# alinjar1996/manipulator_mujoco

Measured on NVIDIA B200. Metric: rollout env-steps/sec (CEM iteration, UR5e+Hand-E scene, 4096 samples x 100 steps per GPU), higher is better.
Workload: dtype f32

## Files before the change

### manipulator_mujoco_b200/csrc/rollout_core.h

```cpp
#pragma once
#include "kmodel.h"
#include "warp_dsl.h"

#ifndef CEMK_SYNC_EVERY
#define CEMK_SYNC_EVERY 1
#endif
#define KM_NC_FAST (KW == 16 ? 20 : 24)
#define KM_NPASS (KM_MAXRPAIR / KW)
#define KM_NC_TOT 48
#define KM_OVF_STRIDE 80
#define KM_NC_BIG 48
#ifndef CEMK_ROW_UNROLL
#define CEMK_ROW_UNROLL 1
#endif
constexpr int kRowUnroll = CEMK_ROW_UNROLL;
#define MJ_MINVAL 1e-15f
#define MJ_MINIMP 0.0001f
#define MJ_MAXIMP 0.9999f

struct LaneRegs {
  float cost_c;
  int nact, off;
  int actmask;
  int farprev;
  int tri;
  float acc[9];
  float h[KM_NV];
#ifdef CEMK_EMU
  float hrow[KM_NV];
#endif
  float td;
  float f0, f1, f2;
};

template <int NC>
struct WarpSmemT {
  static constexpr int NROW = KM_NL + 4 * NC;
  float qpos[16], qvel[12], warm[12];
  float lpos[KM_NL][4], lquat[KM_NL][4], lmat[KM_NL][12];
  float cdof[KM_NL][8];
  float bmat[12];
  float Mr[KM_NL][KM_NL];
  union {
    struct { float capA[KM_MAXCAP][4], capB[KM_MAXCAP][4]; };
    float H[KM_NV][KM_NV];
  };
  float fs[12], as[12], qacc[12], Ma[12], grad[12], search[12];
  int ncon, nrow, nlim, flags;
  union {
    struct { float cinert[KM_NL][12], crb[KM_NL][12], cvel[KM_NL][8], cdofdot[KM_NL][8], cfrc[KM_NL][8]; };
    struct { float rD[NROW], rAref[NROW], rJaref[NROW], rJv[NROW]; };
    struct {
      unsigned short nlist[KM_MAXNEAR];
      float nprev[(KM_MAXSBOX + 1) * KW][2];
    };
  };
  float cgeo[NC][16];
  union {
    float cJ[NC][36];
    struct {
      float bstage[KM_MAXBPAIR][4][4], bnrm[KM_MAXBPAIR][4];
      union {
        struct { float bbR[12], bbc[4], bbsz[2][4], bbrf[4][4], bben[4][4], bbpoly[2][8][4], bbpref[8][4]; };
        struct { float estage[KW][16], eres[KW][8]; };
      };
    };
  };
  float cd[2][NC][3];
  int limdof[KM_NL];
  float limsign[KM_NL];
  float* ovf;
  float* ovf_pad;

  template <bool SP> KMEM float* geo(int c) const { return (!SP || c < NC) ? const_cast<float*>(cgeo[c]) : ovf + (c - NC) * KM_OVF_STRIDE; }
  template <bool SP> KMEM float* jac(int c) const { return (!SP || c < NC) ? const_cast<float*>(cJ[c]) : ovf + (c - NC) * KM_OVF_STRIDE + 16; }
  template <bool SP> KMEM float* dots(int set, int c) const {
    return (!SP || c < NC) ? const_cast<float*>(cd[set][c]) : ovf + (c - NC) * KM_OVF_STRIDE + 52 + 3 * set;
  }
  template <bool SP> KMEM float& row(const float* arr, int off, int r, int nl) const {
    const int rc = r - nl;
    return (!SP || rc < 4 * NC) ? const_cast<float*>(arr)[r] : ovf[((rc >> 2) - NC) * KM_OVF_STRIDE + off + (rc & 3)];
  }
  template <bool SP> KMEM float& D(int r, int nl) const { return row<SP>(rD, 58, r, nl); }
  template <bool SP> KMEM float& Aref(int r, int nl) const { return row<SP>(rAref, 62, r, nl); }
  template <bool SP> KMEM float& Jaref(int r, int nl) const { return row<SP>(rJaref, 66, r, nl); }
  template <bool SP> KMEM float& Jv(int r, int nl) const { return row<SP>(rJv, 70, r, nl); }
};

typedef WarpCtx<LaneRegs> Warp;

KFN int tri_entries(int lane) {
  int tri = 0;
  for (int q = 0; q < 32 / KW; ++q) {
    int e = lane + KW * q, i = 0, j = e;
    if (e < KM_NL * (KM_NL + 1) / 2) { while (j > i) { j -= i + 1; ++i; } } else { i = 15; j = 15; }
    tri |= (i | (j << 4)) << (8 * q);
  }
  return tri;
}
KFN void cold_warp(Warp& W, int bar, int nthr) {
#ifdef CEMK_EMU
  std::memset((void*)&W, 0, sizeof(Warp));
  W.race = g_emu_race;
  for (int l = 0; l < KW; ++l) W.regs[l].tri = tri_entries(l);
  (void)bar; (void)nthr;
#else
  W.lane = threadIdx.x & (KW - 1);
  W.shift = (threadIdx.x & 31) & ~(KW - 1);
  W.mask = KW_FULL << W.shift;
  W.bar = bar; W.nthr = nthr;
  W.regs.tri = tri_entries(W.lane);
#ifdef CEMK_PHASE_TIMING
  W.phase = 0; W.t0 = clock64(); W.stepflag = 0; W.nflag = 0;
  for (int i = 0; i < 24; ++i) { W.ph[i] = 0; W.phs[i] = 0; W.phc[i] = 0; }
  for (int i = 0; i < 24; ++i) W.ev[i] = 0;
#endif
#endif
}

KFN float dot3(const float* a, const float* b) { return a[0] * b[0] + a[1] * b[1] + a[2] * b[2]; }
KFN void cross3(float* r, const float* a, const float* b) {
  float x = a[1] * b[2] - a[2] * b[1], y = a[2] * b[0] - a[0] * b[2], z = a[0] * b[1] - a[1] * b[0];
  r[0] = x; r[1] = y; r[2] = z;
}
KFN void sub3(float* r, const float* a, const float* b) { r[0] = a[0] - b[0]; r[1] = a[1] - b[1]; r[2] = a[2] - b[2]; }
KFN void add3(float* r, const float* a, const float* b) { r[0] = a[0] + b[0]; r[1] = a[1] + b[1]; r[2] = a[2] + b[2]; }
KFN void madd3(float* r, const float* a, const float* b, float s) { r[0] = a[0] + s * b[0]; r[1] = a[1] + s * b[1]; r[2] = a[2] + s * b[2]; }
KFN void copy3(float* r, const float* a) { r[0] = a[0]; r[1] = a[1]; r[2] = a[2]; }
KFN float normalize3(float* a) {
  float n = sqrtf(dot3(a, a));
  if (n > 0.f) { float i = 1.f / n; a[0] *= i; a[1] *= i; a[2] *= i; } else { a[0] = a[1] = a[2] = 0.f; }
  return n;
}
KFN void mat_vec(float* r, const float* m, const float* v) {
  float x = m[0] * v[0] + m[1] * v[1] + m[2] * v[2], y = m[3] * v[0] + m[4] * v[1] + m[5] * v[2], z = m[6] * v[0] + m[7] * v[1] + m[8] * v[2];
  r[0] = x; r[1] = y; r[2] = z;
}
KFN void matT_vec(float* r, const float* m, const float* v) {
  float x = m[0] * v[0] + m[3] * v[1] + m[6] * v[2], y = m[1] * v[0] + m[4] * v[1] + m[7] * v[2], z = m[2] * v[0] + m[5] * v[1] + m[8] * v[2];
  r[0] = x; r[1] = y; r[2] = z;
}
KFN void quat_mul(float* r, const float* a, const float* b) {
  float w = a[0] * b[0] - a[1] * b[1] - a[2] * b[2] - a[3] * b[3];
  float x = a[0] * b[1] + a[1] * b[0] + a[2] * b[3] - a[3] * b[2];
  float y = a[0] * b[2] - a[1] * b[3] + a[2] * b[0] + a[3] * b[1];
  float z = a[0] * b[3] + a[1] * b[2] - a[2] * b[1] + a[3] * b[0];
  r[0] = w; r[1] = x; r[2] = y; r[3] = z;
// ... 173 lines not shown
      sub3(dv, sp.a, nb);
      const float d2 = dot3(dv, dv);
      if (d1 < d2) copy3(sp.a, na); else copy3(sp.b, nb);
    }
    float dir[3];
    sub3(dir, sp.a, sp.b);
    const bool deg = dot3(dir, dir) < 1e-6f;
    const float ed = normalize3(dir);
    const bool front = (eu * dir[u] < 0.f) && (ew * dir[w] < 0.f);
    const float epen = (!deg && front) ? r - ed : -1.f;
    if (epen > bpen) { bpen = epen; bdeg = deg; copy3(beax, dir); copy3(bec, sp.a); copy3(bcc, sp.b); }
  }
  const bool parallel = fabsf(dot3(beax, n)) > 0.99f && !bdeg;
  const bool has_edge = bpen > 0.f && (minface > 0.f ? bpen < minface : true) && !parallel;
  CapBoxEdge out;
  out.pen = has_edge ? bpen : 0.f;
#pragma unroll
  for (int q = 0; q < 3; ++q) { out.pos[q] = 0.5f * (bec[q] + bcc[q] + beax[q] * r); out.nrm[q] = beax[q]; }
  return out;
}
template <bool FULL, bool EDGES = true>
KFN int capsule_box_near(const float* a, const float* b, float r, const float* bsize, CapBoxOut& o, float* nface = nullptr) {
  float bests = fminf(a[0], b[0]) - bsize[0]; int bk = 0; float sg = 1.f;
  { float s = -fmaxf(a[0], b[0]) - bsize[0]; if (s > bests) { bests = s; sg = -1.f; } }
  { float s = fminf(a[1], b[1]) - bsize[1]; if (s > bests) { bests = s; bk = 1; sg = 1.f; } }
  { float s = -fmaxf(a[1], b[1]) - bsize[1]; if (s > bests) { bests = s; bk = 1; sg = -1.f; } }
  { float s = fminf(a[2], b[2]) - bsize[2]; if (s > bests) { bests = s; bk = 2; sg = 1.f; } }
  { float s = -fmaxf(a[2], b[2]) - bsize[2]; if (s > bests) { bests = s; bk = 2; sg = -1.f; } }
  float ak, au, aw, bk_, bu, bw, sk, su, sw;
  if (bk == 0)      { ak = a[0]; au = a[1]; aw = a[2]; bk_ = b[0]; bu = b[1]; bw = b[2]; sk = bsize[0]; su = bsize[1]; sw = bsize[2]; }
  else if (bk == 1) { ak = a[1]; au = a[2]; aw = a[0]; bk_ = b[1]; bu = b[2]; bw = b[0]; sk = bsize[1]; su = bsize[2]; sw = bsize[0]; }
  else              { ak = a[2]; au = a[0]; aw = a[1]; bk_ = b[2]; bu = b[0]; bw = b[1]; sk = bsize[2]; su = bsize[0]; sw = bsize[1]; }
  float t0 = 0.f, t1 = 1.f; bool both = false;
  {
    const float Lu = 2.f * sw, Lw = 2.f * su;
#define CEMK_CLIP(pa, pb, s, tau, L) { \
      float na_ = ((tau) * (pa) - (s)) * (L), nb_ = ((tau) * (pb) - (s)) * (L); \
      bool fa = na_ > 1e-6f, fb = nb_ > 1e-6f; \
      float den = (tau) * ((pb) - (pa)) * (L); \
      float tt = (-na_) / (den + (den == 0.f ? 1e-6f : 0.f)); \
      tt = fminf(fmaxf(tt, 0.f), 1.f); \
      if (fa) t0 = fmaxf(t0, tt); \
      if (fb) t1 = fminf(t1, tt); \
      both = both || (fa && fb); }
    CEMK_CLIP(au, bu, su, -1.f, Lu)
    CEMK_CLIP(aw, bw, sw, -1.f, Lw)
    CEMK_CLIP(au, bu, su, 1.f, Lu)
    CEMK_CLIP(aw, bw, sw, 1.f, Lw)
#undef CEMK_CLIP
  }
  bool mask = !both;
  if (!mask) { t0 = 0.f; t1 = 1.f; }
  {
    const float dk = bk_ - ak, du = bu - au, dw = bw - aw;
    if ((t1 - t0) * (dk * dk + du * du + dw * dw) < 0.f) mask = false;
  }
  const float h0 = sg * (ak + t0 * (bk_ - ak)) - r - sk, h1 = sg * (ak + t1 * (bk_ - ak)) - r - sk;
  o.dist[0] = mask ? h0 : 1.f;
  o.dist[1] = mask ? h1 : 1.f;
  const float nx = bk == 0 ? sg : 0.f, ny = bk == 1 ? sg : 0.f, nz = bk == 2 ? sg : 0.f;
  const int nout = ((fmaxf(a[0], b[0]) > bsize[0] || fminf(a[0], b[0]) < -bsize[0]) ? 1 : 0) +
                   ((fmaxf(a[1], b[1]) > bsize[1] || fminf(a[1], b[1]) < -bsize[1]) ? 1 : 0) +
                   ((fmaxf(a[2], b[2]) > bsize[2] || fminf(a[2], b[2]) < -bsize[2]) ? 1 : 0);
  if (FULL || nout >= 2) {
    const float l0[3] = {sg * (sk + 0.5f * h0), au + t0 * (bu - au), aw + t0 * (bw - aw)};
    const float l1[3] = {sg * (sk + 0.5f * h1), au + t1 * (bu - au), aw + t1 * (bw - aw)};
    if (bk == 0)      { o.pos[0][0] = l0[0]; o.pos[0][1] = l0[1]; o.pos[0][2] = l0[2]; o.pos[1][0] = l1[0]; o.pos[1][1] = l1[1]; o.pos[1][2] = l1[2]; }
    else if (bk == 1) { o.pos[0][1] = l0[0]; o.pos[0][2] = l0[1]; o.pos[0][0] = l0[2]; o.pos[1][1] = l1[0]; o.pos[1][2] = l1[1]; o.pos[1][0] = l1[2]; }
    else              { o.pos[0][2] = l0[0]; o.pos[0][0] = l0[1]; o.pos[0][1] = l0[2]; o.pos[1][2] = l1[0]; o.pos[1][0] = l1[1]; o.pos[1][1] = l1[2]; }
    o.nrm[0][0] = o.nrm[1][0] = -nx; o.nrm[0][1] = o.nrm[1][1] = -ny; o.nrm[0][2] = o.nrm[1][2] = -nz;
    if (EDGES && nout >= 2) {
      const CapBoxEdge e = capbox_edges(a[0], a[1], a[2], b[0], b[1], b[2], r, bsize[0], bsize[1], bsize[2], nx, ny, nz, fminf(-o.dist[0], -o.dist[1]));
      if (e.pen > 0.f) { o.dist[0] = -e.pen; copy3(o.pos[0], e.pos); copy3(o.nrm[0], e.nrm); }
    }
  }
  if (nface) { nface[0] = nx; nface[1] = ny; nface[2] = nz; }
  return nout;
}
struct EdgeEval { float epen, deg, dir[3], pa[3], pb[3]; };
KFN float pick3(const float* v, int k) { return k == 0 ? v[0] : (k == 1 ? v[1] : v[2]); }
KFN void unpick3(float* out, int k, int u, float vk, float vu, float vw) {
  out[0] = k == 0 ? vk : (u == 0 ? vu : vw); out[1] = k == 1 ? vk : (u == 1 ? vu : vw); out[2] = k == 2 ? vk : (u == 2 ? vu : vw);
}
KFN EdgeEval capbox_edge_lane(int e, const float* a, const float* b, float r, const float* bsize) {
  EdgeEval out;
  out.epen = -1.f; out.deg = 0.f;
  out.dir[0] = out.dir[1] = out.dir[2] = 0.f; out.pa[0] = out.pa[1] = out.pa[2] = 0.f; out.pb[0] = out.pb[1] = out.pb[2] = 0.f;
  const int k = e >> 2, u = k == 2 ? 0 : k + 1, w = k == 0 ? 2 : k - 1;
  const float eu = (e & 2) ? 1.f : -1.f, ew = (e & 1) ? 1.f : -1.f;
  const float ak = pick3(a, k), au = pick3(a, u), aw = pick3(a, w), bk = pick3(b, k), bu = pick3(b, u), bw = pick3(b, w);
  const float sk = pick3(bsize, k), su = pick3(bsize, u), sw = pick3(bsize, w);
  const float lou = fminf(au, bu), hiu = fmaxf(au, bu), low = fminf(aw, bw), hiw = fmaxf(aw, bw), lok = fminf(ak, bk), hik = fmaxf(ak, bk);
  const float cu = eu * su, cw = ew * sw;
  const float fu = eu > 0.f ? hiu - cu : cu - lou, fw = ew > 0.f ? hiw - cw : cw - low;
  const float gu = eu > 0.f ? lou - cu : cu - hiu, gw = ew > 0.f ? low - cw : cw - hiw;
  if (!(fu > 0.f && fw > 0.f && gu < r && gw < r && lok < sk + r && hik > -sk - r)) return out;
  const float abk = bk - ak, abu = bu - au, abw = bw - aw;
  const float den = abk * abk + abu * abu + abw * abw + 1e-6f;
  float dv[3] = {abk, abu, abw};
  const float hb = 0.5f * normalize3(dv);
  const float mk = ak + dv[0] * hb, mu = au + dv[1] * hb, mw = aw + dv[2] * hb;
  const float trk = -mk, tru = cu - mu, trw = cw - mw;
  const float dd = dv[0], dat = trk, dbt = dv[0] * trk + dv[1] * tru + dv[2] * trw;
  float ta = (-dat + dd * dbt) / (1.f - dd * dd + 1e-6f);
  float tb = dbt + ta * dd;
  ta = fminf(fmaxf(ta, -sk), sk);
  tb = fminf(fmaxf(tb, -hb), hb);
  float pa[3] = {ta, cu, cw}, pb[3] = {mk + dv[0] * tb, mu + dv[1] * tb, mw + dv[2] * tb};
  float t1 = ((pb[0] + sk) * (2.f * sk)) / (4.f * sk * sk + 1e-6f);
  t1 = fminf(fmaxf(t1, 0.f), 1.f);
  const float na[3] = {-sk + 2.f * sk * t1, cu, cw};
  float d[3];
  sub3(d, pb, na);
  const float d1 = dot3(d, d);
  float t2 = ((pa[0] - ak) * abk + (pa[1] - au) * abu + (pa[2] - aw) * abw) / den;
  t2 = fminf(fmaxf(t2, 0.f), 1.f);
  const float nb[3] = {ak + abk * t2, au + abu * t2, aw + abw * t2};
  sub3(d, pa, nb);
  const float d2 = dot3(d, d);
  if (d1 < d2) copy3(pa, na); else copy3(pb, nb);
  float dir[3];
  sub3(dir, pa, pb);
  const bool deg = dot3(dir, dir) < 1e-6f;
  const float ed = normalize3(dir);
  const bool front = (eu * dir[1] < 0.f) && (ew * dir[2] < 0.f);
  out.epen = (!deg && front) ? r - ed : -1.f;
  out.deg = deg ? 1.f : 0.f;
  unpick3(out.dir, k, u, dir[0], dir[1], dir[2]);
  unpick3(out.pa, k, u, pa[0], pa[1], pa[2]);
  unpick3(out.pb, k, u, pb[0], pb[1], pb[2]);
  return out;
}
template <bool FULL>
KFN void capsule_box(const float* A, const float* B, float r, const float* bpos, const float* bmat, const float* bsize, Contact2& c) {
  float a[3], b[3];
  capbox_local(A, B, bpos, bmat, a, b);
  c.dist[0] = 1.f; c.dist[1] = 1.f;
  if (capbox_far(a, b, r, bsize)) {
    if (FULL) { for (int j = 0; j < 2; ++j) { copy3(c.pos[j], bpos); c.nrm[j][0] = 1.f; c.nrm[j][1] = 0.f; c.nrm[j][2] = 0.f; } }
    return;
  }
  CapBoxOut o;
  capsule_box_near<FULL>(a, b, r, bsize, o);
  c.dist[0] = o.dist[0]; c.dist[1] = o.dist[1];
  if (FULL) {
#pragma unroll
    for (int j = 0; j < 2; ++j) {
      float w[3];
      mat_vec(w, bmat, o.pos[j]); add3(c.pos[j], w, bpos);
      mat_vec(c.nrm[j], bmat, o.nrm[j]);
      normalize3(c.nrm[j]);
    }
  }
}

KFN void manifold_points(int n, float poly[][3], const bool* mask, const float* nrm, int* idx) {
  float dm[16];
  for (int i = 0; i < n; ++i) dm[i] = mask[i] ? 0.f : -1e6f;
  int a = 0;
  for (int i = 1; i < n; ++i) if (dm[i] > dm[a]) a = i;
  int b = 0; float bv = 0.f;
  for (int i = 0; i < n; ++i) { float t[3]; sub3(t, poly[a], poly[i]); float v = dot3(t, t) + dm[i]; if (i == 0 || v > bv) { bv = v; b = i; } }
  float ab[3], t[3];
  sub3(t, poly[a], poly[b]); cross3(ab, nrm, t);
  int c = 0; float cv = 0.f;
  for (int i = 0; i < n; ++i) { float ap[3]; sub3(ap, poly[a], poly[i]); float v = fabsf(dot3(ap, ab)) + dm[i]; if (i == 0 || v > cv) { cv = v; c = i; } }
  float ac[3], bc[3];
  sub3(t, poly[a], poly[c]); cross3(ac, nrm, t);
  sub3(t, poly[b], poly[c]); cross3(bc, nrm, t);
  int dsel = 0; float dv = 0.f;
  for (int i = 0; i < n; ++i) {
    float bp[3], ap[3];
    sub3(bp, poly[b], poly[i]); sub3(ap, poly[a], poly[i]);
    float v = fmaxf(fabsf(dot3(bp, bc)), fabsf(dot3(ap, ac))) + dm[i] - ((i == a || i == b || i == c) ? 2e6f : 0.f);
    if (i == 0 || v > dv) { dv = v; dsel = i; }
  }
  idx[0] = a; idx[1] = b; idx[2] = c; idx[3] = dsel;
}
KFN void box_face(const float* s, int f, float v[4][3], float* n) {
  int k = f >> 1, u = (k + 1) % 3, w = (k + 2) % 3;
  float sg = (f & 1) ? -1.f : 1.f;
  n[0] = n[1] = n[2] = 0.f; n[k] = sg;
  const float su[4] = {-1.f, 1.f, 1.f, -1.f}, sw[4] = {-1.f, -1.f, 1.f, 1.f};
  for (int i = 0; i < 4; ++i) {
    int ii = (f & 1) ? 3 - i : i;
    v[i][k] = sg * s[k]; v[i][u] = su[ii] * s[u]; v[i][w] = sw[ii] * s[w];
  }
}
KNOINLINE int plane_box(const float* ppos, const float* pn, const float* bpos, const float* bmat, const float* bs, float out[4][4]) {
  float v[8][3], sup[8], t[3], pl[3], n[3], smax = -1e30f;
  bool mask[8]; int idx[4];
  sub3(t, ppos, bpos); matT_vec(pl, bmat, t); matT_vec(n, bmat, pn);
  for (int i = 0; i < 8; ++i) {
    v[i][0] = (i & 4 ? 1.f : -1.f) * bs[0]; v[i][1] = (i & 2 ? 1.f : -1.f) * bs[1]; v[i][2] = (i & 1 ? 1.f : -1.f) * bs[2];
    sub3(t, pl, v[i]); sup[i] = dot3(t, n); smax = fmaxf(smax, sup[i]);
  }
  float thr = fmaxf(0.f, smax - 1e-3f);
  for (int i = 0; i < 8; ++i) mask[i] = sup[i] > thr;
  manifold_points(8, v, mask, n, idx);
  int nact = 0;
  for (int k = 0; k < 4; ++k) {
    bool uniq = true;
    for (int q = 0; q < k; ++q) if (idx[q] == idx[k]) uniq = false;
    float w[3];
    mat_vec(w, bmat, v[idx[k]]); add3(w, w, bpos);
    float d = uniq ? -sup[idx[k]] : 1.f;
    madd3(out[k], w, pn, -0.5f * d);
    out[k][3] = d;
    nact += d < 0.f;
  }
  return nact;
}
template <int NC>
KNOINLINE void bb_edge_edge(WarpSmemT<NC>& S, bool act, int slot, int bl, float bn0, float bn1, float bn2, const float* s1, const float* s2,
                            const float* m2, const float* p2) {
// ... 981 lines not shown
      int rem = nearbits & ~R.farprev;
      if (rem) { pf0 = KFFS(rem) - 1; rem &= rem - 1; pf = 1; q00 = pd[(2 * pf0) * KW]; q01 = pd[(2 * pf0 + 1) * KW]; }
      if (rem) { pf1 = KFFS(rem) - 1; pf = 2; q10 = pd[(2 * pf1) * KW]; q11 = pd[(2 * pf1 + 1) * KW]; }
    }
    if (!io.first) {
#pragma unroll 1
      for (int rem = farbits & ~R.farprev; rem; rem &= rem - 1) {
        const int p = KFFS(rem) - 1;
        cc += fmaxf((1.f - 0.005f) * pd[(2 * p) * KW] - 1.f, 0.f) + fmaxf((1.f - 0.005f) * pd[(2 * p + 1) * KW] - 1.f, 0.f);
      }
    }
    if (io.collision_row) {
#pragma unroll 1
      for (int rem = farbits; rem; rem &= rem - 1) {
        const int sl = KP_SLOT(m.rp[(KFFS(rem) - 1) * KW + lane]);
        io.collision_row[sl] = 1.f; io.collision_row[sl + 1] = 1.f;
      }
    }
    R.off = nearbits | ((nearbits & R.farprev) << 16);
    R.farprev = farbits;
    float pv0 = 0.f, pv1 = 0.f;
    if (!io.first) { pv0 = pd[(2 * m.ncbpass) * KW]; pv1 = pd[(2 * m.ncbpass + 1) * KW]; }
#pragma unroll 1
    for (int p = m.ncbpass; p < KM_NPASS; ++p) {
      const int e = p * KW + lane;
      const int x = m.rp[e], ty = KP_TYPE(x);
      const float prev0 = pv0, prev1 = pv1;
      if (!io.first && p + 1 < KM_NPASS) { pv0 = pd[(2 * p + 2) * KW]; pv1 = pd[(2 * p + 3) * KW]; }
      if (ty == KP_NONE) continue;
      const int a = KP_A(x), b = KP_B(x);
      float d0, d1 = 1.f;
      Contact2 c;
      if (ty == KP_CAP_CAP) {
        capsule_capsule<false>(S.capA[a], S.capB[a], m.cap_r[a], S.capA[b], S.capB[b], m.cap_r[b], c);
        d0 = c.dist[0];
      } else {
        plane_capsule<false>(m.plane_pos, m.plane_n, S.capA[b], S.capB[b], m.cap_r[b], c);
        d0 = c.dist[0]; d1 = c.dist[1];
      }
      const int ns = ty == KP_CAP_CAP ? 1 : 2;
      if (d0 < 0.f) { ++nact; actmask |= 1 << (2 * p); cc += 1.f; }
      if (!io.first) cc += fmaxf((1.f - 0.005f) * prev0 - d0, 0.f);
      pd[(2 * p) * KW] = d0;
      if (ns == 2) {
        if (d1 < 0.f) { ++nact; actmask |= 1 << (2 * p + 1); cc += 1.f; }
        if (!io.first) cc += fmaxf((1.f - 0.005f) * prev1 - d1, 0.f);
        pd[(2 * p + 1) * KW] = d1;
      }
      if (io.collision_row) {
        io.collision_row[KP_SLOT(x)] = d0;
        if (ns == 2) io.collision_row[KP_SLOT(x) + 1] = d1;
      }
    }
    R.cost_c += cc;
    if (pf >= 1) { S.nprev[pf0 * KW + lane][0] = q00; S.nprev[pf0 * KW + lane][1] = q01; }
    if (pf >= 2) { S.nprev[pf1 * KW + lane][0] = q10; S.nprev[pf1 * KW + lane][1] = q11; }
    R.acc[6] = __int_as_float((pf >= 1 ? 1 << pf0 : 0) | (pf >= 2 ? 1 << pf1 : 0));
    R.acc[7] = __int_as_float(actmask);
    R.acc[8] = __int_as_float(nact);
  END_LANES
  PHASE(W, 20);
  int ncbcon = 0;
  {
    int ntot = warp_excl_scan(W, [](int, LaneRegs& R) { return KPOPC(R.off & 0xffff); }, [](int, LaneRegs& R, int o) { R.actmask = o; });
    EVENT(W, 0, 1); EVENT(W, 1, ntot > 0); EVENT(W, 2, ntot); EVENT(W, 11, warp_any_groups(W, ntot > 0));
#ifdef CEMK_X_NONEAR
    ntot = 0;
#endif
    if (warp_any_groups(W, ntot > 0)) {
      LANES(W, R)
        int o = R.actmask;
#pragma unroll 1
        for (int rem = R.off & 0xffff; rem; rem &= rem - 1, ++o) {
          const int p = KFFS(rem) - 1;
          S.nlist[o] = (unsigned short)((p * KW + lane) | (((__float_as_int(R.acc[6]) >> p) & 1) << 14) | (((R.off >> (16 + p)) & 1) << 15));
        }
      END_LANES
      PHASE(W, 21);
#pragma unroll 1
      for (int i0 = 0; warp_any_groups(W, i0 < ntot); i0 += KW) {
        const long long tk0 = TICK(); (void)tk0;
        LANES(W, R)
          const int i = i0 + lane;
          R.nact = 0;
          if (i < ntot) {
            const int e = S.nlist[i] & 0x3fff, x = m.rp[e], a = KP_A(x), b = KP_B(x);
            const bool st = b < m.nsbox;
            const float* bsz = st ? m.sb_size[b] : m.fb_size;
            float la[3], lb[3], nf[3];
            CapBoxOut c;
            capbox_local(S.capA[a], S.capB[a], st ? m.sb_pos[b] : S.qpos + KM_NL, st ? m.sb_mat[b] : S.bmat, la, lb);
            const int nout = capsule_box_near<true, false>(la, lb, m.cap_r[a], bsz, c, nf);
#pragma unroll
            for (int k = 0; k < 3; ++k) { R.h[k] = c.pos[0][k]; R.h[3 + k] = c.nrm[0][k]; R.h[6 + k] = c.pos[1][k]; R.h[9 + k] = c.nrm[1][k]; }
            R.f0 = c.dist[0]; R.f1 = c.dist[1];
            if (nout >= 2) {
              R.nact = 1;
              float* g = S.estage[lane];
              g[0] = la[0]; g[1] = la[1]; g[2] = la[2]; g[3] = lb[0]; g[4] = lb[1]; g[5] = lb[2];
              g[6] = bsz[0]; g[7] = bsz[1]; g[8] = bsz[2]; g[9] = m.cap_r[a]; g[10] = nf[0]; g[11] = nf[1]; g[12] = nf[2];
            }
          }
        END_LANES
        const unsigned emine = warp_ballot(W, [](int, LaneRegs& R) { return R.nact != 0; });
#pragma unroll 1
        for (unsigned rem = warp_or_groups(W, emine); rem != 0u; rem &= rem - 1u) {
          const int q = KFFS(rem) - 1;
          const bool mine = (emine >> q) & 1u;
          LANES(W, R)
            R.f2 = -INFINITY;
            if (mine && lane < 12) {
              const float* g = S.estage[q];
              const EdgeEval e1 = capbox_edge_lane(lane, g, g + 3, g[9], g + 6);
              R.f2 = e1.epen;
              if (e1.epen > 0.f) {
                R.acc[0] = e1.dir[0]; R.acc[1] = e1.dir[1]; R.acc[2] = e1.dir[2];
                R.acc[3] = 0.5f * (e1.pa[0] + e1.pb[0] + e1.dir[0] * g[9]); R.acc[4] = 0.5f * (e1.pa[1] + e1.pb[1] + e1.dir[1] * g[9]);
                R.acc[5] = 0.5f * (e1.pa[2] + e1.pb[2] + e1.dir[2] * g[9]);
              }
            }
          END_LANES
          const int bl = warp_argmax_first(W, [](int, LaneRegs& R) { return R.f2; });
          LANES(W, R)
            if (mine && lane == bl) {
              float* g = S.eres[q];
              g[0] = R.f2;
              if (R.f2 > 0.f) { g[1] = R.acc[0]; g[2] = R.acc[1]; g[3] = R.acc[2]; g[4] = R.acc[3]; g[5] = R.acc[4]; g[6] = R.acc[5]; }
            }
          END_LANES
        }
        LANES(W, R)
          const int i = i0 + lane;
          const bool edges = R.nact != 0;
          R.nact = 0;
          if (i < ntot) {
            const int e = S.nlist[i] & 0x3fff, x = m.rp[e], a = KP_A(x), b = KP_B(x);
            const bool wasfar = (S.nlist[i] >> 15) != 0, pref = ((S.nlist[i] >> 14) & 1) != 0, st = b < m.nsbox;
            const float* bpos = st ? m.sb_pos[b] : S.qpos + KM_NL;
            const float* bmat = st ? m.sb_mat[b] : S.bmat;
            if (edges) {
              const float* g = S.eres[lane];
              const float* nf = S.estage[lane] + 10;
              const float bpen = g[0], minface = fminf(-R.f0, -R.f1);
              if (bpen > 0.f) {
                const bool parallel = fabsf(g[1] * nf[0] + g[2] * nf[1] + g[3] * nf[2]) > 0.99f;
                if ((minface > 0.f ? bpen < minface : true) && !parallel) {
                  R.f0 = -bpen;
                  R.h[0] = g[4]; R.h[1] = g[5]; R.h[2] = g[6]; R.h[3] = g[1]; R.h[4] = g[2]; R.h[5] = g[3];
                }
              }
            }
            const float d0 = R.f0, d1 = R.f1;
            float cc = (d0 < 0.f ? 1.f : 0.f) + (d1 < 0.f ? 1.f : 0.f);
            float* pd = io.prevd + (2 * (e / KW)) * KW + (e & (KW - 1));
            if (!io.first) {
              const float prev0 = wasfar ? 1.f : (pref ? S.nprev[e][0] : pd[0]), prev1 = wasfar ? 1.f : (pref ? S.nprev[e][1] : pd[KW]);
              cc += fmaxf((1.f - 0.005f) * prev0 - d0, 0.f) + fmaxf((1.f - 0.005f) * prev1 - d1, 0.f);
            }
            pd[0] = d0; pd[KW] = d1;
            if (io.collision_row) { io.collision_row[KP_SLOT(x)] = d0; io.collision_row[KP_SLOT(x) + 1] = d1; }
            R.cost_c += cc;
            R.nact = (d0 < 0.f ? 1 : 0) + (d1 < 0.f ? 2 : 0);
#ifdef CEMK_X_NEARNOCON
            R.nact = 0;
#endif
            if (R.nact) {
#pragma unroll
              for (int j = 0; j < 2; ++j) {
                const float pj[3] = {R.h[6 * j], R.h[6 * j + 1], R.h[6 * j + 2]}, nj[3] = {R.h[6 * j + 3], R.h[6 * j + 4], R.h[6 * j + 5]};
                float w[3], nw[3];
                mat_vec(w, bmat, pj); add3(w, w, bpos);
                mat_vec(nw, bmat, nj);
                normalize3(nw);
                R.h[6 * j] = w[0]; R.h[6 * j + 1] = w[1]; R.h[6 * j + 2] = w[2];
                R.h[6 * j + 3] = nw[0]; R.h[6 * j + 4] = nw[1]; R.h[6 * j + 5] = nw[2];
              }
              R.f2 = m.cap_invw[a] + (st ? 0.f : m.fb_invw);
              R.tri = (R.tri & 0xffff) | (m.cap_link[a] << 16) | ((st ? 15 : KM_NL) << 20);
            }
          }
        END_LANES
        const long long tk1 = TICK(); (void)tk1;
        EVENT(W, 14, (int)(tk1 - tk0));
        const int nnew = warp_excl_scan(W, [](int, LaneRegs& R) { return (R.nact & 1) + (R.nact >> 1); }, [](int, LaneRegs& R, int o) { R.actmask = o; });
        if (warp_any_groups(W, nnew > 0)) {
          LANES(W, R)
            if (R.nact) {
              const int l1 = (R.tri >> 16) & 15, l2raw = (R.tri >> 20) & 15, l2 = l2raw == 15 ? -1 : l2raw;
              int o = ncbcon + R.actmask;
              if (R.nact & 1) { put_contact<NC>(S, o, R.h, R.h + 3, nullptr, R.f0, R.f2, l1, l2); ++o; }
              if (R.nact & 2) put_contact<NC>(S, o, R.h + 6, R.h + 9, nullptr, R.f1, R.f2, l1, l2);
            }
          END_LANES
        }
        ncbcon += nnew;
        EVENT(W, 15, (int)(TICK() - tk1));
      }
      PHASE(W, 22);
    }
  }
  PHASE(W, 23);
  PHASE_ALIGN(4);
  PHASE(W, 5);
  if (m.has_box) {
    const float* bp = S.qpos + KM_NL;
    LANES(W, R)
      for (int sl = lane; sl < 4 * m.nbpair; sl += KW) S.bstage[sl >> 2][sl & 3][3] = 1.f;
    END_LANES
    const unsigned cand = warp_ballot(W, [&](int q, LaneRegs&) {
      if (q >= m.nbpair) return false;
      if (m.bp_type[q] == KB_PLANE_BOX) {
        const float rb = sqrtf(m.fb_size[0] * m.fb_size[0] + m.fb_size[1] * m.fb_size[1] + m.fb_size[2] * m.fb_size[2]);
        float t[3]; sub3(t, bp, m.plane_pos);
        return dot3(t, m.plane_n) < rb;
      }
      const int a = m.bp_a[q];
      bool overlap = true;
      for (int i = 0; i < 3; ++i) {
        const float ea = fabsf(m.sb_mat[a][3 * i]) * m.sb_size[a][0] + fabsf(m.sb_mat[a][3 * i + 1]) * m.sb_size[a][1] + fabsf(m.sb_mat[a][3 * i + 2]) * m.sb_size[a][2];
        const float eb = fabsf(S.bmat[3 * i]) * m.fb_size[0] + fabsf(S.bmat[3 * i + 1]) * m.fb_size[1] + fabsf(S.bmat[3 * i + 2]) * m.fb_size[2];
        if (fabsf(bp[i] - m.sb_pos[a][i]) > ea + eb) overlap = false;
      }
      return overlap;
    });
#pragma unroll 1
    for (unsigned rem = warp_or_groups(W, cand); rem != 0u; rem &= rem - 1u) {
      EVENT(W, 10, 1);
      const int q = KFFS(rem) - 1;
      const bool mine = (cand >> q) & 1u;
      const int ty = m.bp_type[q], a = m.bp_a[q];
      if (ty == KB_PLANE_BOX) {
        LANES(W, R)
          if (mine && lane == q) { plane_box(m.plane_pos, m.plane_n, bp, S.bmat, m.fb_size, S.bstage[q]); copy3(S.bnrm[q], m.plane_n); }
        END_LANES
      } else {
        const bool sw = ty == KB_BOX_BOX_SWAP;
        box_box_warp<NC>(W, S, mine, q, sw ? bp : m.sb_pos[a], sw ? S.bmat : m.sb_mat[a], sw ? m.fb_size : m.sb_size[a],
                         sw ? m.sb_pos[a] : bp, sw ? m.sb_mat[a] : S.bmat, sw ? m.sb_size[a] : m.fb_size);
      }
    }
  }
  LANES(W, R)
    R.actmask = __float_as_int(R.acc[7]);
    R.nact = __float_as_int(R.acc[8]);
  END_LANES
  const int nrob = ncbcon + warp_excl_scan(W, [](int, LaneRegs& R) { return R.nact; }, [&](int, LaneRegs& R, int o) { R.off = ncbcon + o; });
  const unsigned bmask = m.has_box ? warp_ballot32(W, [&](int l) { return l < 4 * m.nbpair && S.bstage[l >> 2][l & 3][3] < 0.f; }) : 0u;
  const int ncon_all = nrob + KPOPC(bmask);
  const int ncon = ncon_all < KM_NC_TOT ? ncon_all : KM_NC_TOT;
  EVENT(W, 3, ncon); EVENT(W, 4, nrob > 0); EVENT(W, 12, warp_any_groups(W, nrob > 0));
  FLAGSTEP(W, warp_any_groups(W, nrob > 0));
  PHASE(W, 6);
  LANES(W, R)
#ifndef CEMK_X_NOEMIT
    if (R.nact > 0) emit_robot_contacts<NC>(m, S, lane, R.actmask, R.off);
#endif
    for (int sl = lane; sl < 32; sl += KW) {
      if (!(bmask & (1u << sl))) continue;
      const int o = nrob + KPOPC(bmask & ((1u << sl) - 1u)), q = sl >> 2;
      if (o < KM_NC_TOT) {
        const bool sw = m.bp_type[q] == KB_BOX_BOX_SWAP;
        const float* st = S.bstage[q][sl & 3];
        auto put = [&](float* g) {
          copy3(g, st); copy3(g + 3, S.bnrm[q]);
          make_tangents(S.bnrm[q], g + 6, g + 9);
          g[12] = st[3]; g[13] = m.fb_invw; g[14] = sw ? (float)KM_NL : -1.f; g[15] = sw ? -1.f : (float)KM_NL;
        };
        if (o < NC) put(S.cgeo[o]); else put(S.template geo<true>(o));
      }
    }
  END_LANES
  PHASE(W, 18);
  PHASE_ALIGN(2);
  PHASE(W, 7);
  LANES(W, R)
    R.nact = 0;
    if (lane < KM_NL && m.l_limited[lane]) {
// ... 133 lines not shown
```

Measured before the change: 142.6 million.

## Compact capsule-box edge tests into a warp-wide work list instead of per-pair loop

Before, edge evaluation looped serially over each capsule-box pair needing edges and used 12 lanes per pair plus an argmax reduction. Now each lane first computes a 12-bit mask of edges that pass a cheap per-axis prefilter. An exclusive scan packs the surviving (pair, edge) items into a shared list so full warps evaluate them in batches, and each owner lane reduces its own results. Contact emission is also folded into the main lane pass rather than run as a separate one. This cuts idle lanes and serial iterations at the cost of extra shared memory for the index list and a serial per-lane reduction.

```diff
diff --git a/manipulator_mujoco_b200/csrc/rollout_core.h b/manipulator_mujoco_b200/csrc/rollout_core.h
--- a/manipulator_mujoco_b200/csrc/rollout_core.h
+++ b/manipulator_mujoco_b200/csrc/rollout_core.h
@@ -62,7 +62,10 @@
       float bstage[KM_MAXBPAIR][4][4], bnrm[KM_MAXBPAIR][4];
       union {
         struct { float bbR[12], bbc[4], bbsz[2][4], bbrf[4][4], bben[4][4], bbpoly[2][8][4], bbpref[8][4]; };
-        struct { float estage[KW][16], eres[KW][8]; };
+        struct {
+          float estage[KW][16], eres[KW][8];
+          unsigned short eidx[KW * 12];
+        };
       };
     };
   };
@@ -402,6 +405,7 @@
 KFN void unpick3(float* out, int k, int u, float vk, float vu, float vw) {
   out[0] = k == 0 ? vk : (u == 0 ? vu : vw); out[1] = k == 1 ? vk : (u == 1 ? vu : vw); out[2] = k == 2 ? vk : (u == 2 ? vu : vw);
 }
+template <bool TEST = true>
 KFN EdgeEval capbox_edge_lane(int e, const float* a, const float* b, float r, const float* bsize) {
   EdgeEval out;
   out.epen = -1.f; out.deg = 0.f;
@@ -414,7 +418,7 @@
   const float cu = eu * su, cw = ew * sw;
   const float fu = eu > 0.f ? hiu - cu : cu - lou, fw = ew > 0.f ? hiw - cw : cw - low;
   const float gu = eu > 0.f ? lou - cu : cu - hiu, gw = ew > 0.f ? low - cw : cw - hiw;
-  if (!(fu > 0.f && fw > 0.f && gu < r && gw < r && lok < sk + r && hik > -sk - r)) return out;
+  if (TEST && !(fu > 0.f && fw > 0.f && gu < r && gw < r && lok < sk + r && hik > -sk - r)) return out;
   const float abk = bk - ak, abu = bu - au, abw = bw - aw;
   const float den = abk * abk + abu * abu + abw * abw + 1e-6f;
   float dv[3] = {abk, abu, abw};
@@ -451,6 +455,23 @@
   unpick3(out.pb, k, u, pb[0], pb[1], pb[2]);
   return out;
 }
+KFN int capbox_edge_mask(const float* a, const float* b, float r, const float* bsize) {
+  int face = 0, along = 0;
+#pragma unroll
+  for (int j = 0; j < 3; ++j) {
+    const float lo = fminf(a[j], b[j]), hi = fmaxf(a[j], b[j]), s = bsize[j], cn = -1.f * s;
+    if (hi - s > 0.f && lo - s < r) face |= 2 << (2 * j);
+    if (cn - lo > 0.f && cn - hi < r) face |= 1 << (2 * j);
+    if (lo < s + r && hi > -s - r) along |= 1 << j;
+  }
+  int mask = 0;
+#pragma unroll
+  for (int e = 0; e < 12; ++e) {
+    const int k = e >> 2, u = k == 2 ? 0 : k + 1, w = k == 0 ? 2 : k - 1;
+    if (((along >> k) & 1) && ((face >> (2 * u + ((e >> 1) & 1))) & 1) && ((face >> (2 * w + (e & 1))) & 1)) mask |= 1 << e;
+  }
+  return mask;
+}
 template <bool FULL>
 KFN void capsule_box(const float* A, const float* B, float r, const float* bpos, const float* bmat, const float* bsize, Contact2& c) {
   float a[3], b[3];
@@ -1598,7 +1619,8 @@
         const long long tk0 = TICK(); (void)tk0;
         LANES(W, R)
           const int i = i0 + lane;
-          R.nact = 0;
+          R.off = 0;
+          R.f2 = -1.f;
           if (i < ntot) {
             const int e = S.nlist[i] & 0x3fff, x = m.rp[e], a = KP_A(x), b = KP_B(x);
             const bool st = b < m.nsbox;
@@ -1611,61 +1633,75 @@
             for (int k = 0; k < 3; ++k) { R.h[k] = c.pos[0][k]; R.h[3 + k] = c.nrm[0][k]; R.h[6 + k] = c.pos[1][k]; R.h[9 + k] = c.nrm[1][k]; }
             R.f0 = c.dist[0]; R.f1 = c.dist[1];
             if (nout >= 2) {
-              R.nact = 1;
+              R.off = capbox_edge_mask(la, lb, m.cap_r[a], bsz);
               float* g = S.estage[lane];
               g[0] = la[0]; g[1] = la[1]; g[2] = la[2]; g[3] = lb[0]; g[4] = lb[1]; g[5] = lb[2];
               g[6] = bsz[0]; g[7] = bsz[1]; g[8] = bsz[2]; g[9] = m.cap_r[a]; g[10] = nf[0]; g[11] = nf[1]; g[12] = nf[2];
             }
           }
         END_LANES
-        const unsigned emine = warp_ballot(W, [](int, LaneRegs& R) { return R.nact != 0; });
-#pragma unroll 1
-        for (unsigned rem = warp_or_groups(W, emine); rem != 0u; rem &= rem - 1u) {
-          const int q = KFFS(rem) - 1;
-          const bool mine = (emine >> q) & 1u;
+        const int nitem = warp_excl_scan(W, [](int, LaneRegs& R) { return KPOPC(R.off); }, [](int, LaneRegs& R, int o) { R.actmask = o; });
+        if (warp_any_groups(W, nitem > 0)) {
           LANES(W, R)
-            R.f2 = -INFINITY;
-            if (mine && lane < 12) {
-              const float* g = S.estage[q];
-              const EdgeEval e1 = capbox_edge_lane(lane, g, g + 3, g[9], g + 6);
-              R.f2 = e1.epen;
-              if (e1.epen > 0.f) {
-                R.acc[0] = e1.dir[0]; R.acc[1] = e1.dir[1]; R.acc[2] = e1.dir[2];
-                R.acc[3] = 0.5f * (e1.pa[0] + e1.pb[0] + e1.dir[0] * g[9]); R.acc[4] = 0.5f * (e1.pa[1] + e1.pb[1] + e1.dir[1] * g[9]);
-                R.acc[5] = 0.5f * (e1.pa[2] + e1.pb[2] + e1.dir[2] * g[9]);
+            int it = R.actmask;
+#pragma unroll 1
+            for (int rem = R.off; rem; rem &= rem - 1, ++it) S.eidx[it] = (unsigned short)((lane << 4) | (KFFS(rem) - 1));
+          END_LANES
+#pragma unroll 1
+          for (int base = 0; warp_any_groups(W, base < nitem); base += KW) {
+            LANES(W, R)
+              const int it = base + lane;
+              if (it < nitem) {
+                const int q = S.eidx[it] >> 4;
+                const float* g = S.estage[q];
+                const EdgeEval e1 = capbox_edge_lane<false>(S.eidx[it] & 15, g, g + 3, g[9], g + 6);
+                float* o = S.eres[lane];
+                o[0] = e1.epen;
+                if (e1.epen > 0.f) {
+                  o[1] = e1.dir[0]; o[2] = e1.dir[1]; o[3] = e1.dir[2];
+                  o[4] = 0.5f * (e1.pa[0] + e1.pb[0] + e1.dir[0] * g[9]); o[5] = 0.5f * (e1.pa[1] + e1.pb[1] + e1.dir[1] * g[9]);
+                  o[6] = 0.5f * (e1.pa[2] + e1.pb[2] + e1.dir[2] * g[9]);
+                }
               }
-            }
-          END_LANES
-          const int bl = warp_argmax_first(W, [](int, LaneRegs& R) { return R.f2; });
-          LANES(W, R)
-            if (mine && lane == bl) {
-              float* g = S.eres[q];
-              g[0] = R.f2;
-              if (R.f2 > 0.f) { g[1] = R.acc[0]; g[2] = R.acc[1]; g[3] = R.acc[2]; g[4] = R.acc[3]; g[5] = R.acc[4]; g[6] = R.acc[5]; }
-            }
-          END_LANES
+            END_LANES
+            LANES(W, R)
+              const int lo = R.actmask > base ? R.actmask : base, end = R.actmask + KPOPC(R.off);
+#pragma unroll 1
+              for (int it = lo; it < end && it < base + KW; ++it) {
+                const float* o = S.eres[it - base];
+                if (o[0] > R.f2) {
+                  R.f2 = o[0];
+                  if (o[0] > 0.f) { R.acc[0] = o[1]; R.acc[1] = o[2]; R.acc[2] = o[3]; R.acc[3] = o[4]; R.acc[4] = o[5]; R.acc[5] = o[6]; }
+                }
+              }
+              if (end > base && end <= base + KW && R.f2 > 0.f) {
+                const float* nf = S.estage[lane] + 10;
+                const float bpen = R.f2, minface = fminf(-R.f0, -R.f1);
+                const bool parallel = fabsf(R.acc[0] * nf[0] + R.acc[1] * nf[1] + R.acc[2] * nf[2]) > 0.99f;
+                if ((minface > 0.f ? bpen < minface : true) && !parallel) {
+                  R.f0 = -bpen;
+                  R.h[0] = R.acc[3]; R.h[1] = R.acc[4]; R.h[2] = R.acc[5]; R.h[3] = R.acc[0]; R.h[4] = R.acc[1]; R.h[5] = R.acc[2];
+                }
+              }
+            END_LANES
+          }
         }
+        RLANES(W, R)
+          R.nact = i0 + lane < ntot ? (R.f0 < 0.f ? 1 : 0) + (R.f1 < 0.f ? 2 : 0) : 0;
+#ifdef CEMK_X_NEARNOCON
+          R.nact = 0;
+#endif
+        END_RLANES
+        const long long tk1 = TICK(); (void)tk1;
+        EVENT(W, 14, (int)(tk1 - tk0));
+        const int nnew = warp_excl_scan(W, [](int, LaneRegs& R) { return (R.nact & 1) + (R.nact >> 1); }, [](int, LaneRegs& R, int o) { R.actmask = o; });
         LANES(W, R)
           const int i = i0 + lane;
-          const bool edges = R.nact != 0;
-          R.nact = 0;
           if (i < ntot) {
             const int e = S.nlist[i] & 0x3fff, x = m.rp[e], a = KP_A(x), b = KP_B(x);
             const bool wasfar = (S.nlist[i] >> 15) != 0, pref = ((S.nlist[i] >> 14) & 1) != 0, st = b < m.nsbox;
             const float* bpos = st ? m.sb_pos[b] : S.qpos + KM_NL;
             const float* bmat = st ? m.sb_mat[b] : S.bmat;
-            if (edges) {
-              const float* g = S.eres[lane];
-              const float* nf = S.estage[lane] + 10;
-              const float bpen = g[0], minface = fminf(-R.f0, -R.f1);
-              if (bpen > 0.f) {
-                const bool parallel = fabsf(g[1] * nf[0] + g[2] * nf[1] + g[3] * nf[2]) > 0.99f;
-                if ((minface > 0.f ? bpen < minface : true) && !parallel) {
-                  R.f0 = -bpen;
-                  R.h[0] = g[4]; R.h[1] = g[5]; R.h[2] = g[6]; R.h[3] = g[1]; R.h[4] = g[2]; R.h[5] = g[3];
-                }
-              }
-            }
             const float d0 = R.f0, d1 = R.f1;
             float cc = (d0 < 0.f ? 1.f : 0.f) + (d1 < 0.f ? 1.f : 0.f);
             float* pd = io.prevd + (2 * (e / KW)) * KW + (e & (KW - 1));
@@ -1676,10 +1712,6 @@
             pd[0] = d0; pd[KW] = d1;
             if (io.collision_row) { io.collision_row[KP_SLOT(x)] = d0; io.collision_row[KP_SLOT(x) + 1] = d1; }
             R.cost_c += cc;
-            R.nact = (d0 < 0.f ? 1 : 0) + (d1 < 0.f ? 2 : 0);
-#ifdef CEMK_X_NEARNOCON
-            R.nact = 0;
-#endif
             if (R.nact) {
 #pragma unroll
               for (int j = 0; j < 2; ++j) {
@@ -1691,24 +1723,14 @@
                 R.h[6 * j] = w[0]; R.h[6 * j + 1] = w[1]; R.h[6 * j + 2] = w[2];
                 R.h[6 * j + 3] = nw[0]; R.h[6 * j + 4] = nw[1]; R.h[6 * j + 5] = nw[2];
               }
-              R.f2 = m.cap_invw[a] + (st ? 0.f : m.fb_invw);
-              R.tri = (R.tri & 0xffff) | (m.cap_link[a] << 16) | ((st ? 15 : KM_NL) << 20);
+              const float invw = m.cap_invw[a] + (st ? 0.f : m.fb_invw);
+              const int l1 = m.cap_link[a], l2 = st ? -1 : KM_NL;
+              int o = ncbcon + R.actmask;
+              if (R.nact & 1) { put_contact<NC>(S, o, R.h, R.h + 3, nullptr, d0, invw, l1, l2); ++o; }
+              if (R.nact & 2) put_contact<NC>(S, o, R.h + 6, R.h + 9, nullptr, d1, invw, l1, l2);
             }
           }
         END_LANES
-        const long long tk1 = TICK(); (void)tk1;
-        EVENT(W, 14, (int)(tk1 - tk0));
-        const int nnew = warp_excl_scan(W, [](int, LaneRegs& R) { return (R.nact & 1) + (R.nact >> 1); }, [](int, LaneRegs& R, int o) { R.actmask = o; });
-        if (warp_any_groups(W, nnew > 0)) {
-          LANES(W, R)
-            if (R.nact) {
-              const int l1 = (R.tri >> 16) & 15, l2raw = (R.tri >> 20) & 15, l2 = l2raw == 15 ? -1 : l2raw;
-              int o = ncbcon + R.actmask;
-              if (R.nact & 1) { put_contact<NC>(S, o, R.h, R.h + 3, nullptr, R.f0, R.f2, l1, l2); ++o; }
-              if (R.nact & 2) put_contact<NC>(S, o, R.h + 6, R.h + 9, nullptr, R.f1, R.f2, l1, l2);
-            }
-          END_LANES
-        }
         ncbcon += nnew;
         EVENT(W, 15, (int)(TICK() - tk1));
       }
```

After: 147.1 million (median of 6 runs). 1.03x the previous value.
